# bramtoula/multi_robot_SLAM_separators

Measured on AMD Instinct MI355X. Metric: candidate keyframe-pair verifications/sec (NetVLAD NN + ORB match + RANSAC) @1/2/4/8 GPU, higher is better.
Workload: dtype u8+f16+f32+f64

## Files before the change

multi_robot_slam_separators_amd/csrc/k_ransac.hip:

```cpp
#include "sf_device_math.hpp"
#include "sf_internal.hpp"
#include "k_ba.hip"

namespace {

struct RansacLds {
  float4* src;
  float4* dst;
  float* d2;
  uint8_t* mask_a;
  uint8_t* mask_b;
  double* red;
  unsigned long long* sums;
  int* misc;
  float* hyp;
  int* hyp_cnt;
  float* best;
  float* bc;
  uint32_t* cidx;
};

__device__ __forceinline__ RansacLds ransac_carve(unsigned char* p, int kcap) {
  RansacLds L;
  L.src = (float4*)p; p += (size_t)kcap * 16;
  L.dst = (float4*)p; p += (size_t)kcap * 16;
  L.red = (double*)p; p += 64 * 8;
  L.sums = (unsigned long long*)p; p += 4 * 8;
  L.d2 = (float*)p; p += (size_t)kcap * 4;
  L.misc = (int*)p; p += 16 * 4;
  L.mask_a = p; p += kcap;
  L.mask_b = p; p += kcap;
  L.hyp = (float*)p; p += 12 * 64 * 4;
  L.hyp_cnt = (int*)p; p += 5 * 64 * 4;
  L.best = (float*)p; p += 16 * 4;
  L.bc = (float*)p; p += 16 * 4;
  L.cidx = (uint32_t*)p;
  return L;
}

__device__ __forceinline__ bool draw_sample(const RansacLds& L, uint64_t seed, uint32_t it, int max_checks,
                                            uint32_t m, double sdt, uint32_t& s0, uint32_t& s1, uint32_t& s2) {
  for (int a = 0; a < max_checks; ++a) {
    sfd::sample_triplet(seed, it, (uint32_t)a, m, s0, s1, s2);
    float4 p0 = L.src[s0], p1 = L.src[s1], p2 = L.src[s2];
    float ax = p1.x - p0.x, ay = p1.y - p0.y, az = p1.z - p0.z;
    float bx = p2.x - p0.x, by = p2.y - p0.y, bz = p2.z - p0.z;
    float cx = p2.x - p1.x, cy = p2.y - p1.y, cz = p2.z - p1.z;
    float da = (ax * ax + ay * ay) + az * az;
    float db = (bx * bx + by * by) + bz * bz;
    float dc = (cx * cx + cy * cy) + cz * cz;
    if ((double)da > sdt && (double)db > sdt && (double)dc > sdt) return true;
  }
  return false;
}

__device__ inline void fit3(const RansacLds& L, uint32_t s0, uint32_t s1, uint32_t s2, float (&coef)[12]) {
  const float4 p[3] = {L.src[s0], L.src[s1], L.src[s2]};
  const float4 q[3] = {L.dst[s0], L.dst[s1], L.dst[s2]};
  const double inv_n = 1.0 / 3.0;
  double mp[3] = {0.0, 0.0, 0.0}, mq[3] = {0.0, 0.0, 0.0};
#pragma unroll
  for (int i = 0; i < 3; ++i) {
    mp[0] += (double)p[i].x; mp[1] += (double)p[i].y; mp[2] += (double)p[i].z;
    mq[0] += (double)q[i].x; mq[1] += (double)q[i].y; mq[2] += (double)q[i].z;
  }
#pragma unroll
  for (int j = 0; j < 3; ++j) { mp[j] *= inv_n; mq[j] *= inv_n; }
  double S[3][3] = {{0.0, 0.0, 0.0}, {0.0, 0.0, 0.0}, {0.0, 0.0, 0.0}};
  double ga = 0.0, gb = 0.0;
#pragma unroll
  for (int i = 0; i < 3; ++i) {
    const double a[3] = {(double)p[i].x - mp[0], (double)p[i].y - mp[1], (double)p[i].z - mp[2]};
    const double b[3] = {(double)q[i].x - mq[0], (double)q[i].y - mq[1], (double)q[i].z - mq[2]};
#pragma unroll
    for (int j = 0; j < 3; ++j)
#pragma unroll
      for (int k = 0; k < 3; ++k) S[j][k] += a[j] * b[k];
    ga += (a[0] * a[0] + a[1] * a[1]) + a[2] * a[2];
    gb += (b[0] * b[0] + b[1] * b[1]) + b[2] * b[2];
  }
  sfd::rigid_from_moments(S, mp, mq, ga, gb, coef);
}

template <int NW>
__device__ inline void fit_masked(const RansacLds& L, int m, const uint8_t* mask, int n_in, int tid) {
  const double inv_n = 1.0 / (double)n_in;
  double s6[6];
  sfd::canon_reduce<6, 16, NW>(m, tid, L.red, s6, [&](int i, double (&a)[6]) {
    if (mask[i]) {
      float4 p = L.src[i], q = L.dst[i];
      a[0] += (double)p.x; a[1] += (double)p.y; a[2] += (double)p.z;
      a[3] += (double)q.x; a[4] += (double)q.y; a[5] += (double)q.z;
    }
  });
  double mp[3] = {s6[0] * inv_n, s6[1] * inv_n, s6[2] * inv_n};
  double mq[3] = {s6[3] * inv_n, s6[4] * inv_n, s6[5] * inv_n};
  double s9[11];
  sfd::canon_reduce<11, 16, NW>(m, tid, L.red, s9, [&](int i, double (&acc)[11]) {
    if (mask[i]) {
      float4 p = L.src[i], q = L.dst[i];
      const double a[3] = {(double)p.x - mp[0], (double)p.y - mp[1], (double)p.z - mp[2]};
      const double b[3] = {(double)q.x - mq[0], (double)q.y - mq[1], (double)q.z - mq[2]};
#pragma unroll
      for (int j = 0; j < 3; ++j)
#pragma unroll
        for (int k = 0; k < 3; ++k) acc[3 * j + k] += a[j] * b[k];
      acc[9] += (a[0] * a[0] + a[1] * a[1]) + a[2] * a[2];
      acc[10] += (b[0] * b[0] + b[1] * b[1]) + b[2] * b[2];
    }
  });
  if (tid < 64) {
    double S[3][3];
#pragma unroll
    for (int j = 0; j < 3; ++j)
#pragma unroll
      for (int k = 0; k < 3; ++k) S[j][k] = s9[3 * j + k];
    float coef[12];
    sfd::rigid_from_moments(S, mp, mq, s9[9], s9[10], coef);
    if (tid < 12) {
      float v = coef[0];
#pragma unroll
      for (int k = 1; k < 12; ++k) v = (tid == k) ? coef[k] : v;
      L.bc[tid] = v;
    }
  }
}

struct SelCounts { int n, low, diff; };

template <int NW>
__device__ inline SelCounts select_within(const RansacLds& L, int m, const float* cf, double thr2, uint8_t* mask,
                                          const uint8_t* prev, double sigma, double thr, int tid) {
  float coef[12];
#pragma unroll
  for (int k = 0; k < 12; ++k) coef[k] = cf[k];
  unsigned long long acc = 0;
  const int m4 = (m + 3) & ~3;
  for (int i = tid; i < m4; i += 64 * NW) {
    float r2 = __int_as_float(0x7F800000);
    if (i < m) {
      float4 p = L.src[i], q = L.dst[i];
      const float v = sfd::residual2(coef, p.x, p.y, p.z, q.x, q.y, q.z);
      const bool in = (double)v < thr2;
      r2 = in ? v : r2;
      const bool was = prev ? prev[i] != 0 : false;
      mask[i] = in ? 1 : 0;
      const bool low = in && !(thr < sigma * sqrt(2.1981 * (double)v));
      acc += (in ? 1ull : 0ull) + (low ? (1ull << 13) : 0ull) + ((was != in) ? (1ull << 26) : 0ull);
    }
    L.d2[i] = r2;
  }
  const int lane = tid & 63, wave = tid >> 6;
#pragma unroll
  for (int off = 32; off >= 1; off >>= 1) acc += __shfl_xor(acc, off);
  __syncthreads();
  if (lane == 0) L.sums[wave] = acc;
  __syncthreads();
  unsigned long long t = L.sums[0];
#pragma unroll
  for (int w = 1; w < NW; ++w) t += L.sums[w];
  SelCounts c;
  c.n = (int)(t & 0x1FFFull);
  c.low = (int)((t >> 13) & 0x1FFFull);
  c.diff = (int)((t >> 26) & 0x1FFFull);
  return c;
}

typedef __attribute__((address_space(3))) const float* lds_cfloat_p;
typedef __attribute__((address_space(3))) unsigned* lds_uint_p;
typedef __attribute__((address_space(3))) int* lds_int_p;
template <int NT>
__device__ __attribute__((noinline)) float radix_select_rank(lds_cfloat_p d2, lds_uint_p hist, lds_int_p misc, int m4,
                                                             int rank, int tid) {
  const int lane = tid & 63, wave = tid >> 6;
  for (int b = tid; b < 4 * 256; b += NT) hist[b] = 0u;
  __syncthreads();
  unsigned prefix = 0u;
#pragma unroll 1
  for (int p = 0; p < 4; ++p) {
    const int shift = 24 - 8 * p;
    for (int i = tid; i < m4; i += NT) {
      const unsigned bits = __float_as_uint(d2[i]);
      if (p == 0 || (bits >> (shift + 8)) == prefix)
        __hip_atomic_fetch_add(&hist[p * 256 + ((bits >> shift) & 255u)], 1u, __ATOMIC_RELAXED, __HIP_MEMORY_SCOPE_WORKGROUP);
    }
    __syncthreads();
    if (wave == 0) {
      const unsigned h0 = hist[p * 256 + 4 * lane], h1 = hist[p * 256 + 4 * lane + 1], h2 = hist[p * 256 + 4 * lane + 2],
                     h3 = hist[p * 256 + 4 * lane + 3];
      const unsigned s = (h0 + h1) + (h2 + h3);
      unsigned incl = s;
#pragma unroll
      for (int off = 1; off < 64; off <<= 1) {
        const unsigned y = __shfl_up(incl, off);
        if (lane >= off) incl += y;
      }
      const unsigned excl = incl - s;
      if (excl <= (unsigned)rank && (unsigned)rank < incl) {
        unsigned r = (unsigned)rank - excl;
        int b = 0;
        if (r >= h0) { r -= h0; b = 1; if (r >= h1) { r -= h1; b = 2; if (r >= h2) { r -= h2; b = 3; } } }
        misc[2] = (int)((prefix << 8) | (unsigned)(4 * lane + b));
        misc[3] = (int)r;
      }
    }
    __syncthreads();
    prefix = (unsigned)misc[2];
    rank = misc[3];
  }
  return __uint_as_float(prefix);
}

template <int NW>
__device__ __forceinline__ double variance_of(const RansacLds& L, int m, int n, int tid) {
  const float medv = radix_select_rank<64 * NW>((lds_cfloat_p)L.d2, (lds_uint_p) reinterpret_cast<unsigned*>(L.hyp),
                                       (lds_int_p)L.misc, (m + 3) & ~3, n >> 1, tid);
  return 2.1981 * (double)medv;
}

template <int R>
__device__ __forceinline__ int count_round(const RansacLds& L, const int* hv, int i0, int i1, int lane, float thr2f) {
  constexpr int G = 64 / R;
  const int h = lane & (R - 1), g = lane / R;
  int cnt = 0;
  if (hv[h]) {
    float coef[12];
#pragma unroll
    for (int k = 0; k < 12; ++k) coef[k] = L.hyp[k * 64 + h];
    int i = i0 + g;
#pragma unroll 1
    for (; i + 3 * G < i1; i += 4 * G) {
      float4 p[4], q[4];
#pragma unroll
      for (int u = 0; u < 4; ++u) { p[u] = L.src[i + u * G]; q[u] = L.dst[i + u * G]; }
#pragma unroll
      for (int u = 0; u < 4; ++u) {
        const float r2 = sfd::residual2(coef, p[u].x, p[u].y, p[u].z, q[u].x, q[u].y, q[u].z);
        cnt += (r2 <= thr2f) ? 1 : 0;
      }
    }
#pragma unroll 1
    for (; i < i1; i += G) {
      const float4 p = L.src[i], q = L.dst[i];
      const float r2 = sfd::residual2(coef, p.x, p.y, p.z, q.x, q.y, q.z);
      cnt += (r2 <= thr2f) ? 1 : 0;
    }
  }
  return cnt;
}

__device__ __forceinline__ int count_own(const RansacLds& L, const float (&coef)[12], int m, float thr2f) {
  int cnt = 0;
  int i = 0;
#pragma unroll 1
  for (; i + 1 < m; i += 2) {
    const float4 p0 = L.src[i], q0 = L.dst[i], p1 = L.src[i + 1], q1 = L.dst[i + 1];
    const float r0 = sfd::residual2(coef, p0.x, p0.y, p0.z, q0.x, q0.y, q0.z);
    const float r1 = sfd::residual2(coef, p1.x, p1.y, p1.z, q1.x, q1.y, q1.z);
    cnt += ((r0 <= thr2f) ? 1 : 0) + ((r1 <= thr2f) ? 1 : 0);
  }
  if (i < m) {
    const float4 p = L.src[i], q = L.dst[i];
    const float r2 = sfd::residual2(coef, p.x, p.y, p.z, q.x, q.y, q.z);
    cnt += (r2 <= thr2f) ? 1 : 0;
  }
  return cnt;
}

struct ScanState {
  int best;
  int best_it;
  int it;
  double k;
};

__device__ __forceinline__ int shfl_up_from(int v, int off, int lane) {
  const int src = lane >= off ? lane - off : lane;
  return __builtin_amdgcn_ds_bpermute(src << 2, v);
}
__device__ __forceinline__ double shfl_up_from(double v, int off, int lane) {
  const int src = lane >= off ? lane - off : lane;
  const long long b = __double_as_longlong(v);
  const int lo = __builtin_amdgcn_ds_bpermute(src << 2, (int)(b & 0xFFFFFFFFll));
  const int hi = __builtin_amdgcn_ds_bpermute(src << 2, (int)(b >> 32));
  return __longlong_as_double(((long long)hi << 32) | (unsigned)lo);
}

__device__ __forceinline__ bool replay_round(const RansacLds& L, ScanState& S, int base, int R, int lane, int c,
                                             bool present, int max_it, bool adaptive, double inv_m,
                                             double log_probability, bool park = true) {
  int x = present ? c : -1;
#pragma unroll
  for (int off = 1; off < 64; off <<= 1) {
    const int y = shfl_up_from(x, off, lane);
    if (lane >= off) x = max(x, y);
  }
  x = max(x, S.best);
  double kj = 1.0;
  if (x >= 0) {
    const double w = (double)x * inv_m;
    double pno = 1.0 - (w * w) * w;
    if (pno < 2.220446049250313e-16) pno = 2.220446049250313e-16;
    if (pno > 1.0 - 2.220446049250313e-16) pno = 1.0 - 2.220446049250313e-16;
    kj = log_probability / sfd::canon_log(pno);
  }
  double kprev = shfl_up_from(kj, 1, lane);
  if (lane == 0) kprev = S.k;
  const int it = base + lane;
  const bool top_ok = present && (!adaptive || (double)it < kprev) && c >= 0;
  const unsigned long long fail = ~__ballot(top_ok);
  const int n_proc = fail ? (__ffsll((long long)fail) - 1) : 64;
  if (n_proc > 0) {
    const int nb = __builtin_amdgcn_readlane(x, n_proc - 1);
    const long long kb = __double_as_longlong(kj);
    const double nk = __longlong_as_double(
        ((long long)__builtin_amdgcn_readlane((int)(kb >> 32), n_proc - 1) << 32) |
        (unsigned)__builtin_amdgcn_readlane((int)(kb & 0xFFFFFFFFll), n_proc - 1));
    if (nb > S.best) {
      const unsigned long long at = __ballot(present && c == nb && lane < n_proc);
      const int lb = __ffsll((long long)at) - 1;
      S.best = nb;
      S.best_it = base + lb;
      if (park && lane < 12) L.best[lane] = L.hyp[lane * 64 + lb];
    }
    S.k = nk;
  }
  S.it = base + n_proc;
  return n_proc < R || base + R > max_it;
}

__host__ __device__ inline size_t sf_ransac_lds_bytes_dev(int kcap) {
  return (size_t)kcap * 32 + 64 * 8 + 4 * 8 + (size_t)kcap * 4 + 16 * 4 + (size_t)kcap * 2 + 12 * 64 * 4 + 5 * 64 * 4 +
         16 * 4 + 16 * 4 + (size_t)kcap * 4;
}

__device__ __forceinline__ void write_null_pass(PassState& out, int matches) {
  PassState ps;
#pragma unroll
  for (int i = 0; i < 12; ++i) ps.T[i] = 0.f;
  ps.var = 1.0; ps.var_ang = 1.0;
  ps.is_null = 1;
  ps.inliers = 0;
  ps.matches = matches;
  ps.pad = 0;
  out = ps;
}

template <int DIR = 0, int NW = 4>
__device__ __forceinline__ void ransac_body(const StoreView& st, int pair, int sF, int sT, const uint32_t* cl, int n_corr,
                                            PassState& out, const DeviceParams& P, unsigned char* lds,
                                            int trace_base = 2, uint8_t* mask_out = nullptr) {
  constexpr int NT = 64 * NW;
  const int tid = (int)threadIdx.x;
  const int lane = tid & 63, wave = tid >> 6;
  const int kcap = st.kcap;
  const RansacLds L = ransac_carve(lds, kcap);

  const float* xF = st.xyz + (size_t)sF * kcap * 3;
  const float* xT = st.xyz + (size_t)sT * kcap * 3;
  if (tid < 16) L.misc[tid] = 0;
  __syncthreads();
  int m = 0;
  for (int base = 0; base < n_corr; base += NT) {
    const int i = base + tid;
    bool ok = false;
    float ax = 0, ay = 0, az = 0, bx = 0, by = 0, bz = 0;
    if (i < n_corr) {
      const uint32_t c = cl[i];
      const float* a = DIR ? xT + 3 * (c >> 16) : xF + 3 * (c & 0xFFFFu);
      const float* b = DIR ? xF + 3 * (c & 0xFFFFu) : xT + 3 * (c >> 16);
      ax = a[0]; ay = a[1]; az = a[2];
      bx = b[0]; by = b[1]; bz = b[2];
      ok = sfd::finite3(ax, ay, az) && sfd::finite3(bx, by, bz) && (ax != 0.f || ay != 0.f || az != 0.f) &&
           (bx != 0.f || by != 0.f || bz != 0.f);
    }
    const unsigned long long bal = __ballot(ok);
    const int before = __popcll(bal & ((1ull << lane) - 1ull));
    if (lane == 0) L.misc[4 + wave] = __popcll(bal);
    __syncthreads();
    int woff = 0, total = 0;
#pragma unroll
    for (int w = 0; w < NW; ++w) {
      int c = L.misc[4 + w];
      if (w < wave) woff += c;
      total += c;
    }
    if (ok) {
      L.src[m + woff + before] = make_float4(ax, ay, az, 0.f);
      L.dst[m + woff + before] = make_float4(bx, by, bz, 0.f);
      L.cidx[m + woff + before] = cl[i];
    }
    m += total;
    __syncthreads();
  }

  SF_TRACE_MARK(P, pair, trace_base + 0);
  if (m < P.min_inliers || m < 3) {
    if (tid == 0) write_null_pass(out, m);
    return;
  }

  const int fit_wave = pair & (NW - 1);

  const double inv_m = 1.0 / (double)m;
  if (tid == 0) reinterpret_cast<double*>(L.sums)[2] = inv_m;
  double sdt = 0.0;
  {
    double mean[3];
    double s3[3];
    sfd::canon_reduce<3, 16, NW>(m, tid, L.red, s3, [&](int i, double (&a)[3]) {
      float4 p = L.src[i];
      a[0] += (double)p.x; a[1] += (double)p.y; a[2] += (double)p.z;
    });
    mean[0] = s3[0] * inv_m; mean[1] = s3[1] * inv_m; mean[2] = s3[2] * inv_m;
    double c6[6];
    sfd::canon_reduce<6, 16, NW>(m, tid, L.red, c6, [&](int i, double (&a)[6]) {
      float4 p = L.src[i];
      const double a0 = (double)p.x - mean[0], a1 = (double)p.y - mean[1], a2 = (double)p.z - mean[2];
      a[0] += a0 * a0; a[1] += a0 * a1; a[2] += a0 * a2;
      a[3] += a1 * a1; a[4] += a1 * a2; a[5] += a2 * a2;
    });
    if (wave == fit_wave) {
      double ev[3];
      sfd::sym3_eigenvalues(c6[0] * inv_m, c6[1] * inv_m, c6[2] * inv_m, c6[3] * inv_m, c6[4] * inv_m, c6[5] * inv_m, ev);
      sdt = ((sqrt(ev[0]) + sqrt(ev[1])) + sqrt(ev[2])) / 3.0;
      sdt = sdt * sdt;
      if (lane == 0) {
        double* st = reinterpret_cast<double*>(L.sums);
        st[0] = sdt;
        st[1] = 1.0;
        L.misc[12] = -1;
        L.misc[13] = -1;
        L.misc[14] = 0;
      }
    }
  }

  if (P.dbg_stop == 1) { if (tid == 0) write_null_pass(out, m); return; }
  SF_TRACE_MARK(P, pair, trace_base + 1);

  const int max_it = P.iterations;
  int* hv = L.hyp_cnt + 4 * 64;
  {
    constexpr int R = 16;
    const int base = 0;
    int lane_r = lane, wave_r = wave;
    asm volatile("" : "+v"(lane_r), "+v"(wave_r));
    const int it = base + lane_r;
    if (wave_r == fit_wave) {
      int valid = 0;
      if (lane_r < R && it <= max_it) {
        uint32_t s0, s1, s2;
        if (draw_sample(L, P.seed, (uint32_t)it, P.max_sample_checks, (uint32_t)m, reinterpret_cast<const double*>(L.sums)[0],
                        s0, s1, s2)) {
          float coef[12];
          fit3(L, s0, s1, s2, coef);
          int lane_s = lane;
          asm volatile("" : "+v"(lane_s));
#pragma unroll
          for (int k = 0; k < 12; ++k) L.hyp[k * 64 + lane_s] = coef[k];
          valid = 1;
        }
      }
      int lane_s = lane;
      asm volatile("" : "+v"(lane_s));
      hv[lane_s] = valid;
    }
    __syncthreads();
    SF_TRACE_MARK(P, pair, trace_base == 2 ? 18 : 21);
    {
      int lane_c = lane, wave_c = wave;
      asm volatile("" : "+v"(lane_c), "+v"(wave_c));
      const double thr2 = P.inlier_thr * P.inlier_thr;
      float thr2f = (float)thr2;
      if ((double)thr2f >= thr2) thr2f = __uint_as_float(__float_as_uint(thr2f) - 1u);
      const int slice = (m + NW - 1) / NW;
      const int i0 = min(m, wave_c * slice), i1 = min(m, i0 + slice);
      L.hyp_cnt[wave_c * 64 + lane_c] = count_round<16>(L, hv, i0, i1, lane_c, thr2f);
    }
    __syncthreads();
    SF_TRACE_MARK(P, pair, trace_base == 2 ? 19 : 22);
    if (wave_r == fit_wave) {
      asm volatile("" : "+v"(lane_r));
      int tot = 0;
      const int h = lane_r & 15;
#pragma unroll
      for (int w = 0; w < NW; ++w)
#pragma unroll
        for (int g = 0; g < 4; ++g) tot += L.hyp_cnt[w * 64 + g * 16 + h];
      const bool present = lane_r < R && it <= max_it;
      const int c = (present && hv[lane_r]) ? tot : -1;
      ScanState S;
      S.best = L.misc[12]; S.best_it = L.misc[13]; S.it = L.misc[14];
      S.k = reinterpret_cast<const double*>(L.sums)[1];
      const bool stop = replay_round(L, S, base, R, lane_r, c, present, max_it, P.adaptive_stop != 0,
                                     reinterpret_cast<const double*>(L.sums)[2],
                                     sfd::canon_log(1.0 - 0.99));
      if (lane_r == 0) {
        L.misc[12] = S.best; L.misc[13] = S.best_it; L.misc[14] = S.it;
        reinterpret_cast<double*>(L.sums)[1] = S.k;
        L.misc[0] = S.best_it;
        L.misc[1] = stop ? 1 : 0;
      }
    }
    __syncthreads();
    SF_TRACE_MARK(P, pair, trace_base == 2 ? 20 : 23);
  }
  if (!L.misc[1]) {
    for (int base = 16; base <= max_it; base += 64 * NW) {
      int lane_r = lane, wave_r = wave;
      asm volatile("" : "+v"(lane_r), "+v"(wave_r));
      const int it = base + 64 * wave_r + lane_r;
      float coef[12];
#pragma unroll
      for (int k = 0; k < 12; ++k) coef[k] = 0.f;
      int cnt = -1;
      if (it <= max_it) {
        uint32_t s0, s1, s2;
        if (draw_sample(L, P.seed, (uint32_t)it, P.max_sample_checks, (uint32_t)m, reinterpret_cast<const double*>(L.sums)[0],
                        s0, s1, s2)) {
          fit3(L, s0, s1, s2, coef);
          const double thr2 = P.inlier_thr * P.inlier_thr;
          float thr2f = (float)thr2;
          if ((double)thr2f >= thr2) thr2f = __uint_as_float(__float_as_uint(thr2f) - 1u);
          cnt = count_own(L, coef, m, thr2f);
        }
      }
      {
        int lane_s = lane, wave_s = wave;
        asm volatile("" : "+v"(lane_s), "+v"(wave_s));
        L.hyp_cnt[wave_s * 64 + lane_s] = cnt;
      }
      __syncthreads();
      if (wave_r == fit_wave) {
        asm volatile("" : "+v"(lane_r));
        ScanState S;
        S.best = L.misc[12]; S.best_it = L.misc[13]; S.it = L.misc[14];
        S.k = reinterpret_cast<const double*>(L.sums)[1];
        bool stop = false;
#pragma unroll 1
        for (int sub = 0; sub < NW && !stop; ++sub) {
          const int b = base + 64 * sub;
          if (b > max_it) break;
          const bool present = b + lane_r <= max_it;
          const int c = present ? L.hyp_cnt[sub * 64 + lane_r] : -1;
          stop = replay_round(L, S, b, 64, lane_r, c, present, max_it, P.adaptive_stop != 0,
                              reinterpret_cast<const double*>(L.sums)[2], sfd::canon_log(1.0 - 0.99), false);
        }
        if (lane_r == 0) {
          L.misc[12] = S.best; L.misc[13] = S.best_it; L.misc[14] = S.it;
          reinterpret_cast<double*>(L.sums)[1] = S.k;
          L.misc[0] = S.best_it;
          L.misc[1] = stop ? 1 : 0;
        }
      }
      __syncthreads();
      if (cnt >= 0 && L.misc[0] == it) {
#pragma unroll
        for (int k = 0; k < 12; ++k) L.best[k] = coef[k];
      }
      __syncthreads();
      if (L.misc[1]) break;
    }
  }
  int tid_b = tid;
  asm volatile("" : "+v"(tid_b));
  if (P.dbg_stop == 2 || P.dbg_stop == 3) { if (tid_b == 0) write_null_pass(out, m); return; }
  SF_TRACE_MARK(P, pair, trace_base + 2);
  const int best_it = L.misc[0];
  if (best_it < 0) {
    if (tid_b == 0) write_null_pass(out, m);
    return;
  }

  const double thr = P.inlier_thr;
  const double thr2 = thr * thr;
  const double sigma = P.refine_sigma;
  SelCounts sc = select_within<NW>(L, m, L.best, thr2, L.mask_a, nullptr, sigma, thr, tid_b);
  int n_inl = sc.n;
  const uint8_t* inl = L.mask_a;
  int n_last = n_inl;
  const float* model = L.best;

  if (P.dbg_stop == 4) { if (tid_b == 0) write_null_pass(out, m); return; }
  SF_TRACE_MARK(P, pair, trace_base + 3);

  if (P.refine_iterations > 0) {
    double error_threshold = thr;
    int refine_iterations = 0;
    bool inlier_changed = false;
    uint8_t* prev = L.mask_a;
    uint8_t* neu = L.mask_b;
    int n_prev = n_inl, n_new = 0;
    for (int i = tid_b; i < m; i += NT) neu[i] = 0;
    if (tid_b < 12) L.bc[tid_b] = L.best[tid_b];
    int n_sizes = 0, z1 = 0, z2 = 0, z3 = 0, z4 = 0;
    do {
      if (n_prev >= 3) fit_masked<NW>(L, m, prev, n_prev, tid_b);
      z4 = z3; z3 = z2; z2 = z1; z1 = n_prev;
      ++n_sizes;
      __syncthreads();
      sc = select_within<NW>(L, m, L.bc, error_threshold * error_threshold, neu, prev, sigma, thr, tid_b);
      n_new = sc.n;
      n_last = n_new;
      if (n_new == 0) {
        ++refine_iterations;
        if (refine_iterations >= P.refine_iterations) break;
        continue;
      }
      if ((n_new >> 1) < sc.low) {
        const double variance = variance_of<NW>(L, m, n_new, tid_b);
        const double sthr = sigma * sqrt(variance);
        error_threshold = thr < sthr ? thr : sthr;
      } else {
        error_threshold = thr;
      }
      inlier_changed = false;
      { uint8_t* t = prev; prev = neu; neu = t; int tn = n_prev; n_prev = n_new; n_new = tn; }
      if (n_new != n_prev) {
        if (n_sizes >= 4 && z1 == z3 && z2 == z4) break;
        inlier_changed = true;
        continue;
      }
      inlier_changed = sc.diff != 0;
    } while (inlier_changed && ++refine_iterations < P.refine_iterations);
    inl = neu;
    n_inl = n_new;
    model = L.bc;
  }

  if (P.dbg_stop == 5) { if (tid_b == 0) write_null_pass(out, m); return; }
  SF_TRACE_MARK(P, pair, trace_base + 4);
  if (n_inl >= 3) {
    if (mask_out)
      for (int i = tid; i < m; i += NT)
        if (inl[i]) mask_out[L.cidx[i] & 0xFFFFu] = 1;
    const double variance = variance_of<NW>(L, m, n_last, tid_b);
    if (tid_b == 0) {
      PassState ps;
#pragma unroll
      for (int i = 0; i < 12; ++i) ps.T[i] = 0.f;
      ps.is_null = 1;
      ps.matches = m;
      ps.pad = 0;
      ps.var = variance;
      ps.var_ang = variance;
      ps.inliers = n_inl;
      if (n_inl >= P.min_inliers) {
        double R9[9], t[3];
#pragma unroll
        for (int i = 0; i < 3; ++i) {
#pragma unroll
          for (int j = 0; j < 3; ++j) R9[3 * i + j] = (double)model[4 * i + j];
          t[i] = (double)model[4 * i + 3];
        }
        bool allz = true;
#pragma unroll
        for (int i = 0; i < 3; ++i) {
#pragma unroll
          for (int j = 0; j < 3; ++j) ps.T[4 * i + j] = (float)R9[3 * j + i];
          ps.T[4 * i + 3] = (float)(-((R9[i] * t[0] + R9[3 + i] * t[1]) + R9[6 + i] * t[2]));
        }
#pragma unroll
        for (int i = 0; i < 12; ++i) allz = allz && (ps.T[i] == 0.f);
        ps.is_null = allz ? 1 : 0;
        if (P.force_3dof && !allz) sfd::to3dof_canon(ps.T);
      }
      out = ps;
    }
  } else if (tid_b == 0) {
    write_null_pass(out, m);
  }
  SF_TRACE_MARK(P, pair, trace_base + 5);
}

__device__ inline void pass_to3dof(PassState& ps, int times) {
  if (ps.is_null) return;
  for (int t = 0; t < times; ++t) sfd::to3dof_canon(ps.T);
}

template <int DIR>
__global__ void __launch_bounds__(SF_BLOCK, 4)
k_ransac(StoreView st, const int32_t* __restrict__ pair_from, const int32_t* __restrict__ pair_to,
         const int32_t* __restrict__ list, const int32_t* __restrict__ counter,
         const uint32_t* __restrict__ corr, const CorrHeader* __restrict__ hdr,
         PassState* __restrict__ pass, uint8_t* __restrict__ mask, int extra_3dof, DeviceParams P) {
  if ((int)blockIdx.x >= *counter) return;
  extern __shared__ __attribute__((aligned(16))) unsigned char smem_raw[];
  const int pair = list[blockIdx.x];
  ransac_body<DIR>(st, pair, pair_from[pair], pair_to[pair], corr + (size_t)pair * st.kcap, hdr[pair].n_corr,
                       pass[pair], P, smem_raw, 2, mask ? mask + (size_t)pair * st.kcap : nullptr);
  if (extra_3dof && threadIdx.x == 0) pass_to3dof(pass[pair], extra_3dof);
}

__global__ void __launch_bounds__(64)
k_merge_directions(const int32_t* __restrict__ list, const int32_t* __restrict__ counter, PassState* __restrict__ fwd,
                   const PassState* __restrict__ back, const uint8_t* __restrict__ mask_f,
                   const uint8_t* __restrict__ mask_b, int kcap, int extra_3dof) {
  if ((int)blockIdx.x >= *counter) return;
  const int pair = list[blockIdx.x], lane = threadIdx.x;
  int uni = 0;
  for (int i = lane; i < kcap; i += 64) uni += (mask_f[(size_t)pair * kcap + i] | mask_b[(size_t)pair * kcap + i]) ? 1 : 0;
#pragma unroll
  for (int off = 32; off >= 1; off >>= 1) uni += __shfl_xor(uni, off);
  if (lane != 0) return;
  PassState a = fwd[pair];
  const PassState b = back[pair];
  a.inliers = uni;
  a.matches = a.matches > b.matches ? a.matches : b.matches;
  if (!b.is_null) {
    float inv[12];
    sfd::rigid_inverse_canon(b.T, inv);
    if (a.is_null) {
#pragma unroll
      for (int i = 0; i < 12; ++i) a.T[i] = inv[i];
      a.is_null = 0;
      a.var = b.var;
      a.var_ang = b.var_ang;
    } else {
      float mid[12];
      sfd::interpolate_half_canon(a.T, inv, mid);
#pragma unroll
      for (int i = 0; i < 12; ++i) a.T[i] = mid[i];
      a.var = (a.var + b.var) / 2.0;
      a.var_ang = (a.var_ang + b.var_ang) / 2.0;
    }
  }
  pass_to3dof(a, extra_3dof);
  fwd[pair] = a;
}

}

size_t sf_ransac_lds_bytes(int kcap, int iterations) {
  (void)iterations;
  return sf_ransac_lds_bytes_dev(kcap);
}

int sf_launch_ransac(sf_context* c, StoreView st, const int32_t* d_from, const int32_t* d_to, int n, int pass) {
  if (n <= 0) return SF_OK;
  const bool ba = c->dparams.bundle_adjustment != 0;
  const size_t lds = (sf_ransac_lds_bytes(st.kcap, c->dparams.iterations) + 15) & ~(size_t)15;
  if (lds > 160 * 1024) return sf_fail(c, SF_ERANGE, "RANSAC workgroup needs %zu B of LDS (> 160 KiB)", lds);
  const bool bidir = c->dparams.bidirectional != 0;
  bool& attr = c->ransac_attr_set;
  if (!attr) {
    SF_HIP(c, hipFuncSetAttribute((const void*)k_ransac<0>, hipFuncAttributeMaxDynamicSharedMemorySize, 160 * 1024));
    SF_HIP(c, hipFuncSetAttribute((const void*)k_ransac<1>, hipFuncAttributeMaxDynamicSharedMemorySize, 160 * 1024));
    attr = true;
  }
  int32_t* counters = (int32_t*)c->w->counters.p;
  const int32_t* list = (const int32_t*)(pass == 1 ? c->w->list1.p : c->w->list3.p);
  const int32_t* counter = counters + (pass == 1 ? 0 : 2);
  PassState* ps = (PassState*)(pass == 1 ? c->w->pass1.p : c->w->pass2.p);
  const int end_3dof = c->dparams.force_3dof ? (pass == 1 ? 2 : 1) : 0;
  uint8_t *mask_f = nullptr, *mask_b = nullptr;
  if (bidir) {
    int rc;
    const size_t mb = (size_t)n * st.kcap;
    if ((rc = sf_buf_reserve(c, c->w->dir_mask, 2 * mb)) != SF_OK) return rc;
    if ((rc = sf_buf_reserve(c, c->w->pass_back, (size_t)n * sizeof(PassState))) != SF_OK) return rc;
    mask_f = (uint8_t*)c->w->dir_mask.p;
    mask_b = mask_f + mb;
    SF_HIP(c, hipMemsetAsync(mask_f, 0, 2 * mb, c->stream));
  } else if (ba) {
    int rc;
    const size_t mb = (size_t)n * st.kcap;
    if ((rc = sf_buf_reserve(c, c->w->dir_mask, mb)) != SF_OK) return rc;
    mask_f = (uint8_t*)c->w->dir_mask.p;
    SF_HIP(c, hipMemsetAsync(mask_f, 0, mb, c->stream));
  }
  const int kid = pass == 1 ? SF_K_RANSAC1 : SF_K_RANSAC2;
  sf_prof_begin(c, kid);
  auto launch = [&](auto kern, PassState* out, uint8_t* mask, int extra) {
    hipLaunchKernelGGL(kern, dim3(n), dim3(SF_BLOCK), lds, c->stream, st, d_from, d_to, list, counter,
                       (const uint32_t*)(pass == 1 ? c->w->corr1.p : c->w->corr2.p),
                       (const CorrHeader*)(pass == 1 ? c->w->hdr1.p : c->w->hdr2.p), out, mask, extra, c->dparams);
  };
  if (ba && !bidir) launch(k_ransac<0>, ps, mask_f, 0);
  else if (!bidir) launch(k_ransac<0>, ps, nullptr, end_3dof);
  else {
    launch(k_ransac<0>, ps, mask_f, 0);
    launch(k_ransac<1>, (PassState*)c->w->pass_back.p, mask_b, 0);
    if (ba) {
      const int rc = sf_launch_merge_directions_ba(c, st, d_from, d_to, n, pass, false, mask_f, mask_b);
      if (rc != SF_OK) return rc;
    } else
    hipLaunchKernelGGL(k_merge_directions, dim3(n), dim3(64), 0, c->stream, list, counter, ps,
                       (const PassState*)c->w->pass_back.p, (const uint8_t*)mask_f, (const uint8_t*)mask_b, st.kcap, end_3dof);
  }
  sf_prof_end(c, kid);
  SF_HIP(c, hipGetLastError());
  if (ba && !bidir) return sf_launch_ba_pass(c, st, d_from, d_to, n, pass, pass == 1 ? 1 : 3, mask_f, nullptr, false, nullptr);
  return SF_OK;
}
```

multi_robot_slam_separators_amd/csrc/sf_device_math.hpp:

```cpp
#pragma once
#include <hip/hip_runtime.h>
#include <stdint.h>

namespace sfd {

__device__ __forceinline__ uint64_t mix64(uint64_t z) {
  z += 0x9E3779B97F4A7C15ULL;
  z = (z ^ (z >> 30)) * 0xBF58476D1CE4E5B9ULL;
  z = (z ^ (z >> 27)) * 0x94D049BB133111EBULL;
  return z ^ (z >> 31);
}

__device__ __forceinline__ void sample_triplet(uint64_t seed, uint32_t it, uint32_t attempt, uint32_t m,
                                               uint32_t& i0, uint32_t& i1, uint32_t& i2) {
  uint64_t ha = mix64(seed ^ mix64(((uint64_t)it << 32) | (uint64_t)attempt));
  uint64_t hb = mix64(ha);
  uint32_t r0 = (uint32_t)(ha >> 32), r1 = (uint32_t)ha, r2 = (uint32_t)(hb >> 32);
  i0 = __umulhi(r0, m);
  i1 = __umulhi(r1, m - 1);
  if (i1 >= i0) ++i1;
  i2 = __umulhi(r2, m - 2);
  uint32_t lo = i0 < i1 ? i0 : i1, hi = i0 < i1 ? i1 : i0;
  if (i2 >= lo) ++i2;
  if (i2 >= hi) ++i2;
}

__device__ inline double canon_log(double x) {
  int e;
  double m = frexp(x, &e);
  if (m < 0.70710678118654752440) { m = m * 2.0; e -= 1; }
  double z = (m - 1.0) / (m + 1.0);
  double z2 = z * z;
  double s = 1.0 / 27.0;
#pragma unroll
  for (int k = 12; k >= 0; --k) s = s * z2 + 1.0 / (double)(2 * k + 1);
  return 2.0 * z * s + (double)e * 0.69314718055994530942;
}

template <int N>
__device__ inline void jacobi(double (&a)[N][N], double (&v)[N][N]) {
#pragma unroll
  for (int i = 0; i < N; ++i)
#pragma unroll
    for (int j = 0; j < N; ++j) v[i][j] = (i == j) ? 1.0 : 0.0;
  for (int sweep = 0; sweep < 50; ++sweep) {
    double sm = 0.0;
#pragma unroll
    for (int p = 0; p < N - 1; ++p)
#pragma unroll
      for (int q = p + 1; q < N; ++q) sm += fabs(a[p][q]);
    if (sm == 0.0) break;
#pragma unroll
    for (int p = 0; p < N - 1; ++p) {
#pragma unroll
      for (int q = p + 1; q < N; ++q) {
        double apq = a[p][q];
        double g = 100.0 * fabs(apq);
        double app = fabs(a[p][p]), aqq = fabs(a[q][q]);
        if (sweep > 3 && app + g == app && aqq + g == aqq) {
          a[p][q] = 0.0;
          a[q][p] = 0.0;
        } else if (apq != 0.0) {
          double h = a[q][q] - a[p][p];
          double t;
          if (fabs(h) + g == fabs(h)) {
            t = apq / h;
          } else {
            double theta = 0.5 * h / apq;
            t = 1.0 / (fabs(theta) + sqrt(1.0 + theta * theta));
            if (theta < 0.0) t = -t;
          }
          double c = 1.0 / sqrt(1.0 + t * t);
          double s = t * c;
#pragma unroll
          for (int k = 0; k < N; ++k) {
            double akp = a[k][p], akq = a[k][q];
            a[k][p] = c * akp - s * akq;
            a[k][q] = s * akp + c * akq;
          }
#pragma unroll
          for (int k = 0; k < N; ++k) {
            double apk = a[p][k], aqk = a[q][k];
            a[p][k] = c * apk - s * aqk;
            a[q][k] = s * apk + c * aqk;
          }
          a[p][q] = 0.0;
          a[q][p] = 0.0;
#pragma unroll
          for (int k = 0; k < N; ++k) {
            double vkp = v[k][p], vkq = v[k][q];
            v[k][p] = c * vkp - s * vkq;
            v[k][q] = s * vkp + c * vkq;
          }
        }
      }
    }
  }
}

__device__ __forceinline__ double det3(double a, double b, double c, double d, double e, double f, double g,
                                       double h, double i) {
  return (a * (e * i - f * h) - b * (d * i - f * g)) + c * (d * h - e * g);
}

__device__ inline void sym3_eigenvalues(double c00, double c01, double c02, double c11, double c12, double c22,
                                        double (&ev)[3]) {
  const double c2 = (c00 + c11) + c22;
  const double c1 = ((c00 * c11 - c01 * c01) + (c00 * c22 - c02 * c02)) + (c11 * c22 - c12 * c12);
  const double c0 = det3(c00, c01, c02, c01, c11, c12, c02, c12, c22);
  double x = c2;
  for (int it = 0; it < 50; ++it) {
    const double pv = ((x - c2) * x + c1) * x - c0;
    const double dp = (3.0 * x - 2.0 * c2) * x + c1;
    if (dp == 0.0) break;
    const double xn = x - pv / dp;
    if (!(xn < x)) break;
    const double step = x - xn;
    x = xn;
    if (step <= 1e-14 * fabs(xn)) break;
  }
  const double l1 = x > 0.0 ? x : 0.0;
  const double s = c2 - l1;
  const double q = c1 - l1 * s;
  double disc = s * s - 4.0 * q;
  if (!(disc > 0.0)) disc = 0.0;
  const double r = sqrt(disc);
  double l2 = 0.5 * (s + r), l3 = 0.5 * (s - r);
  if (!(l2 > 0.0)) l2 = 0.0;
  if (!(l3 > 0.0)) l3 = 0.0;
  ev[0] = l1; ev[1] = l2; ev[2] = l3;
}

__device__ inline void rigid_from_moments(const double (&S)[3][3], const double (&mp)[3],
                                          const double (&mq)[3], double ga, double gb, float (&coef)[12]) {
  double Nm[4][4];
  Nm[0][0] = (S[0][0] + S[1][1]) + S[2][2];
  Nm[1][1] = (S[0][0] - S[1][1]) - S[2][2];
  Nm[2][2] = (S[1][1] - S[0][0]) - S[2][2];
  Nm[3][3] = (S[2][2] - S[0][0]) - S[1][1];
  Nm[0][1] = Nm[1][0] = S[1][2] - S[2][1];
  Nm[0][2] = Nm[2][0] = S[2][0] - S[0][2];
  Nm[0][3] = Nm[3][0] = S[0][1] - S[1][0];
  Nm[1][2] = Nm[2][1] = S[0][1] + S[1][0];
  Nm[1][3] = Nm[3][1] = S[2][0] + S[0][2];
  Nm[2][3] = Nm[3][2] = S[1][2] + S[2][1];

  double ss = 0.0;
#pragma unroll
  for (int j = 0; j < 3; ++j)
#pragma unroll
    for (int k = 0; k < 3; ++k) ss += S[j][k] * S[j][k];
  const double c2 = -2.0 * ss;
  const double c1 = -8.0 * det3(S[0][0], S[0][1], S[0][2], S[1][0], S[1][1], S[1][2], S[2][0], S[2][1], S[2][2]);
  const double m0 = det3(Nm[1][1], Nm[1][2], Nm[1][3], Nm[2][1], Nm[2][2], Nm[2][3], Nm[3][1], Nm[3][2], Nm[3][3]);
  const double m1 = det3(Nm[1][0], Nm[1][2], Nm[1][3], Nm[2][0], Nm[2][2], Nm[2][3], Nm[3][0], Nm[3][2], Nm[3][3]);
  const double m2 = det3(Nm[1][0], Nm[1][1], Nm[1][3], Nm[2][0], Nm[2][1], Nm[2][3], Nm[3][0], Nm[3][1], Nm[3][3]);
  const double m3 = det3(Nm[1][0], Nm[1][1], Nm[1][2], Nm[2][0], Nm[2][1], Nm[2][2], Nm[3][0], Nm[3][1], Nm[3][2]);
  const double c0 = ((Nm[0][0] * m0 - Nm[0][1] * m1) + Nm[0][2] * m2) - Nm[0][3] * m3;

  double x = 0.5 * (ga + gb);
  for (int it = 0; it < 50; ++it) {
    const double x2 = x * x;
    const double b = (x2 + c2) * x;
    const double a = b + c1;
    const double pv = a * x + c0;
    const double dp = (2.0 * x2 * x + b) + a;
    if (dp == 0.0) break;
    const double xn = x - pv / dp;
    if (!(xn < x)) break;
    const double step = x - xn;
    x = xn;
    if (step <= 1e-14 * fabs(xn)) break;
  }

  const double b00 = Nm[0][0] - x, b11 = Nm[1][1] - x, b22 = Nm[2][2] - x, b33 = Nm[3][3] - x;
  const double b01 = Nm[0][1], b02 = Nm[0][2], b03 = Nm[0][3], b12 = Nm[1][2], b13 = Nm[1][3], b23 = Nm[2][3];
  const double a00 = det3(b11, b12, b13, b12, b22, b23, b13, b23, b33);
  const double a11 = det3(b00, b02, b03, b02, b22, b23, b03, b23, b33);
  const double a22 = det3(b00, b01, b03, b01, b11, b13, b03, b13, b33);
  const double a33 = det3(b00, b01, b02, b01, b11, b12, b02, b12, b22);
  const double a01 = -det3(b01, b12, b13, b02, b22, b23, b03, b23, b33);
  const double a02 = det3(b01, b11, b13, b02, b12, b23, b03, b13, b33);
  const double a03 = -det3(b01, b11, b12, b02, b12, b22, b03, b13, b23);
  const double a12 = -det3(b00, b01, b03, b02, b12, b23, b03, b13, b33);
  const double a13 = det3(b00, b01, b02, b02, b12, b22, b03, b13, b23);
  const double a23 = -det3(b00, b01, b02, b01, b11, b12, b03, b13, b23);
  double best = fabs(a00);
  double w = a00, qx = a01, qy = a02, qz = a03;
  if (fabs(a11) > best) { best = fabs(a11); w = a01; qx = a11; qy = a12; qz = a13; }
  if (fabs(a22) > best) { best = fabs(a22); w = a02; qx = a12; qy = a22; qz = a23; }
  if (fabs(a33) > best) { best = fabs(a33); w = a03; qx = a13; qy = a23; qz = a33; }
  double nrm2 = ((w * w + qx * qx) + qy * qy) + qz * qz;
  if (!(best > 0.0) || !(nrm2 > 0.0) || !isfinite(nrm2)) {
    const double shift = 0.5 * (ga + gb);
    double v0 = 1.0, v1 = 0.5, v2 = 0.25, v3 = 0.125;
    for (int it = 0; it < 64; ++it) {
      const double u0 = (((Nm[0][0] + shift) * v0 + Nm[0][1] * v1) + Nm[0][2] * v2) + Nm[0][3] * v3;
      const double u1 = ((Nm[0][1] * v0 + (Nm[1][1] + shift) * v1) + Nm[1][2] * v2) + Nm[1][3] * v3;
      const double u2 = ((Nm[0][2] * v0 + Nm[1][2] * v1) + (Nm[2][2] + shift) * v2) + Nm[2][3] * v3;
      const double u3 = ((Nm[0][3] * v0 + Nm[1][3] * v1) + Nm[2][3] * v2) + (Nm[3][3] + shift) * v3;
      const double n2 = ((u0 * u0 + u1 * u1) + u2 * u2) + u3 * u3;
      if (!(n2 > 0.0) || !isfinite(n2)) break;
      const double in = 1.0 / sqrt(n2);
      v0 = u0 * in; v1 = u1 * in; v2 = u2 * in; v3 = u3 * in;
    }
    w = v0; qx = v1; qy = v2; qz = v3;
    nrm2 = ((w * w + qx * qx) + qy * qy) + qz * qz;
  }
  const double inv = 1.0 / sqrt(nrm2);
  w = w * inv;
  const double x_ = qx * inv, y = qy * inv, z = qz * inv;
  const double xx = x_ * x_, yy = y * y, zz = z * z, xy = x_ * y, xz = x_ * z, yz = y * z;
  const double wx = w * x_, wy = w * y, wz = w * z;
  double R[9];
  R[0] = 1.0 - 2.0 * (yy + zz); R[1] = 2.0 * (xy - wz);       R[2] = 2.0 * (xz + wy);
  R[3] = 2.0 * (xy + wz);       R[4] = 1.0 - 2.0 * (xx + zz); R[5] = 2.0 * (yz - wx);
  R[6] = 2.0 * (xz - wy);       R[7] = 2.0 * (yz + wx);       R[8] = 1.0 - 2.0 * (xx + yy);
#pragma unroll
  for (int j = 0; j < 3; ++j) {
    double t = mq[j] - ((R[3 * j] * mp[0] + R[3 * j + 1] * mp[1]) + R[3 * j + 2] * mp[2]);
    coef[4 * j + 0] = (float)R[3 * j + 0];
    coef[4 * j + 1] = (float)R[3 * j + 1];
    coef[4 * j + 2] = (float)R[3 * j + 2];
    coef[4 * j + 3] = (float)t;
  }
}

__device__ __forceinline__ float residual2(const float (&c)[12], float px, float py, float pz,
                                           float qx, float qy, float qz) {
  float tx = __fmaf_rn(c[2], pz, __fmaf_rn(c[1], py, __fmaf_rn(c[0], px, c[3])));
  float ty = __fmaf_rn(c[6], pz, __fmaf_rn(c[5], py, __fmaf_rn(c[4], px, c[7])));
  float tz = __fmaf_rn(c[10], pz, __fmaf_rn(c[9], py, __fmaf_rn(c[8], px, c[11])));
  float dx = tx - qx, dy = ty - qy, dz = tz - qz;
  return __fmaf_rn(dz, dz, __fmaf_rn(dy, dy, dx * dx));
}


template <int C>
__device__ __forceinline__ void sum_stage(double (&w)[32], int& idx, int lane, int off) {
  if constexpr (C > 1) {
    const bool up = (lane & off) != 0;
#pragma unroll
    for (int k = 0; k < C / 2; ++k) {
      const double send = up ? w[k] : w[k + C / 2];
      const double keep = up ? w[k + C / 2] : w[k];
      w[k] = keep + __shfl_xor(send, off);
    }
    idx += up ? C / 2 : 0;
  } else {
    w[0] = w[0] + __shfl_xor(w[0], off);
  }
}

template <int N, int STRIDE>
__device__ __forceinline__ void block_sum_canon(double (&v)[N], double* red, int tid) {
  static_assert(N >= 1 && N <= 32 && STRIDE >= N, "at most 32 values");
  constexpr int P = N <= 1 ? 1 : N <= 2 ? 2 : N <= 4 ? 4 : N <= 8 ? 8 : N <= 16 ? 16 : 32;
  static_assert(STRIDE >= P, "scratch rows must hold the padded count");
  const int lane = tid & 63, wave = tid >> 6;
  double w[32];
#pragma unroll
  for (int k = 0; k < 32; ++k) w[k] = k < N ? v[k] : 0.0;
  int idx = 0;
  sum_stage<P>(w, idx, lane, 32);
  sum_stage<(P / 2 > 1 ? P / 2 : 1)>(w, idx, lane, 16);
  sum_stage<(P / 4 > 1 ? P / 4 : 1)>(w, idx, lane, 8);
  sum_stage<(P / 8 > 1 ? P / 8 : 1)>(w, idx, lane, 4);
  sum_stage<(P / 16 > 1 ? P / 16 : 1)>(w, idx, lane, 2);
  sum_stage<(P / 32 > 1 ? P / 32 : 1)>(w, idx, lane, 1);
  __syncthreads();
  red[wave * STRIDE + idx] = w[0];
  __syncthreads();
#pragma unroll
  for (int k = 0; k < N; ++k) v[k] = ((red[k] + red[STRIDE + k]) + red[2 * STRIDE + k]) + red[3 * STRIDE + k];
}

template <int N, int STRIDE, int NW, class F>
__device__ __forceinline__ void canon_reduce(int m, int tid, double* red, double (&out)[N], F acc) {
  if constexpr (NW == 4) {
#pragma unroll
    for (int k = 0; k < N; ++k) out[k] = 0.0;
    for (int i = tid; i < m; i += 256) acc(i, out);
    block_sum_canon<N, STRIDE>(out, red, tid);
  } else {
    static_assert(NW == 1 || NW == 2, "one, two or four wavefronts");
    constexpr int P = N <= 1 ? 1 : N <= 2 ? 2 : N <= 4 ? 4 : N <= 8 ? 8 : N <= 16 ? 16 : 32;
    static_assert(STRIDE >= P, "scratch rows must hold the padded count");
    const int lane = tid & 63, wave = tid >> 6;
    __syncthreads();
#pragma unroll 1
    for (int j = 0; j < 4 / NW; ++j) {
      const int vw = wave * (4 / NW) + j;
      if (64 * vw >= m) {
        if (lane < P) red[vw * STRIDE + lane] = 0.0;
        continue;
      }
      double w[32];
#pragma unroll
      for (int k = 0; k < 32; ++k) w[k] = 0.0;
      {
        double v[N];
#pragma unroll
        for (int k = 0; k < N; ++k) v[k] = 0.0;
        for (int i = lane + 64 * vw; i < m; i += 256) acc(i, v);
#pragma unroll
        for (int k = 0; k < N; ++k) w[k] = v[k];
      }
      int idx = 0;
      sum_stage<P>(w, idx, lane, 32);
      sum_stage<(P / 2 > 1 ? P / 2 : 1)>(w, idx, lane, 16);
      sum_stage<(P / 4 > 1 ? P / 4 : 1)>(w, idx, lane, 8);
      sum_stage<(P / 8 > 1 ? P / 8 : 1)>(w, idx, lane, 4);
      sum_stage<(P / 16 > 1 ? P / 16 : 1)>(w, idx, lane, 2);
      sum_stage<(P / 32 > 1 ? P / 32 : 1)>(w, idx, lane, 1);
      red[vw * STRIDE + idx] = w[0];
    }
    __syncthreads();
#pragma unroll
    for (int k = 0; k < N; ++k) out[k] = ((red[k] + red[STRIDE + k]) + red[2 * STRIDE + k]) + red[3 * STRIDE + k];
  }
}

template <int N, int STRIDE>
__device__ __forceinline__ void block_sum_canon_to_lds(const double (&v)[N], double* red, double* out, int tid) {
  static_assert(N >= 1 && N <= 32 && STRIDE >= N, "at most 32 values");
  constexpr int P = N <= 1 ? 1 : N <= 2 ? 2 : N <= 4 ? 4 : N <= 8 ? 8 : N <= 16 ? 16 : 32;
  static_assert(STRIDE >= P, "scratch rows must hold the padded count");
  const int lane = tid & 63, wave = tid >> 6;
  double w[32];
#pragma unroll
  for (int k = 0; k < 32; ++k) w[k] = k < N ? v[k] : 0.0;
  int idx = 0;
  sum_stage<P>(w, idx, lane, 32);
  sum_stage<(P / 2 > 1 ? P / 2 : 1)>(w, idx, lane, 16);
  sum_stage<(P / 4 > 1 ? P / 4 : 1)>(w, idx, lane, 8);
  sum_stage<(P / 8 > 1 ? P / 8 : 1)>(w, idx, lane, 4);
  sum_stage<(P / 16 > 1 ? P / 16 : 1)>(w, idx, lane, 2);
  sum_stage<(P / 32 > 1 ? P / 32 : 1)>(w, idx, lane, 1);
  __syncthreads();
  red[wave * STRIDE + idx] = w[0];
  __syncthreads();
  if (tid < N) out[tid] = ((red[tid] + red[STRIDE + tid]) + red[2 * STRIDE + tid]) + red[3 * STRIDE + tid];
  __syncthreads();
}

template <int N, int STRIDE, int NW, bool ONCE = false, class F>
__device__ __forceinline__ void canon_reduce_to_lds(int m, int tid, double* red, double* out, F acc) {
  if constexpr (NW == 4) {
    double v[N];
#pragma unroll
    for (int k = 0; k < N; ++k) v[k] = 0.0;
    if constexpr (ONCE) { if (tid < m) acc(tid, v); }
    else { for (int i = tid; i < m; i += 256) acc(i, v); }
    block_sum_canon_to_lds<N, STRIDE>(v, red, out, tid);
  } else {
    static_assert(NW == 1 || NW == 2, "one, two or four wavefronts");
    constexpr int P = N <= 1 ? 1 : N <= 2 ? 2 : N <= 4 ? 4 : N <= 8 ? 8 : N <= 16 ? 16 : 32;
    static_assert(STRIDE >= P, "scratch rows must hold the padded count");
    const int lane = tid & 63, wave = tid >> 6;
    __syncthreads();
#pragma unroll 1
    for (int j = 0; j < 4 / NW; ++j) {
      const int vw = wave * (4 / NW) + j;
      if (64 * vw >= m) {
        if (lane < P) red[vw * STRIDE + lane] = 0.0;
        continue;
      }
      double w[32];
#pragma unroll
      for (int k = 0; k < 32; ++k) w[k] = 0.0;
      {
        double v[N];
#pragma unroll
        for (int k = 0; k < N; ++k) v[k] = 0.0;
        if constexpr (ONCE) { if (lane + 64 * vw < m) acc(lane + 64 * vw, v); }
        else { for (int i = lane + 64 * vw; i < m; i += 256) acc(i, v); }
#pragma unroll
        for (int k = 0; k < N; ++k) w[k] = v[k];
      }
      int idx = 0;
      sum_stage<P>(w, idx, lane, 32);
      sum_stage<(P / 2 > 1 ? P / 2 : 1)>(w, idx, lane, 16);
      sum_stage<(P / 4 > 1 ? P / 4 : 1)>(w, idx, lane, 8);
      sum_stage<(P / 8 > 1 ? P / 8 : 1)>(w, idx, lane, 4);
      sum_stage<(P / 16 > 1 ? P / 16 : 1)>(w, idx, lane, 2);
      sum_stage<(P / 32 > 1 ? P / 32 : 1)>(w, idx, lane, 1);
      red[vw * STRIDE + idx] = w[0];
    }
    __syncthreads();
    if (tid < N) out[tid] = ((red[tid] + red[STRIDE + tid]) + red[2 * STRIDE + tid]) + red[3 * STRIDE + tid];
    __syncthreads();
  }
}

__device__ __forceinline__ bool finite3(float x, float y, float z) {
  return isfinite(x) && isfinite(y) && isfinite(z);
}

__device__ inline void to3dof_canon(float* T) {
  const double r11 = (double)T[0], r21 = (double)T[4];
  const double h = sqrt(r11 * r11 + r21 * r21);
  float c = 1.0f, s = 0.0f;
  if (h > 0.0) { c = (float)(r11 / h); s = (float)(r21 / h); }
  const float x = T[3], y = T[7];
  T[0] = c; T[1] = -s; T[2] = 0.0f; T[3] = x;
  T[4] = s; T[5] = c; T[6] = 0.0f; T[7] = y;
  T[8] = 0.0f; T[9] = 0.0f; T[10] = 1.0f; T[11] = 0.0f;
}

__device__ inline void quat_from_rot_canon(const float* T, double (&q)[4]) {
  double m[3][3];
#pragma unroll
  for (int i = 0; i < 3; ++i)
#pragma unroll
    for (int j = 0; j < 3; ++j) m[i][j] = (double)T[4 * i + j];
  const double tr = (m[0][0] + m[1][1]) + m[2][2];
  if (tr > 0.0) {
    double t = sqrt(tr + 1.0);
    q[3] = 0.5 * t; t = 0.5 / t;
    q[0] = (m[2][1] - m[1][2]) * t; q[1] = (m[0][2] - m[2][0]) * t; q[2] = (m[1][0] - m[0][1]) * t;
  } else {
    int i = 0;
    if (m[1][1] > m[0][0]) i = 1;
    if (m[2][2] > m[i][i]) i = 2;
    const int j = (i + 1) % 3, k = (j + 1) % 3;
    double t = sqrt(((m[i][i] - m[j][j]) - m[k][k]) + 1.0);
    double qv[3];
    qv[i] = 0.5 * t; t = 0.5 / t;
    q[3] = (m[k][j] - m[j][k]) * t;
    qv[j] = (m[j][i] + m[i][j]) * t;
    qv[k] = (m[k][i] + m[i][k]) * t;
    q[0] = qv[0]; q[1] = qv[1]; q[2] = qv[2];
  }
}

__device__ inline void rigid_inverse_canon(const float* T, float* out) {
  double R[9], t[3];
#pragma unroll
  for (int i = 0; i < 3; ++i) {
#pragma unroll
    for (int j = 0; j < 3; ++j) R[3 * i + j] = (double)T[4 * i + j];
    t[i] = (double)T[4 * i + 3];
  }
#pragma unroll
  for (int i = 0; i < 3; ++i) {
#pragma unroll
    for (int j = 0; j < 3; ++j) out[4 * i + j] = (float)R[3 * j + i];
    out[4 * i + 3] = (float)(-((R[i] * t[0] + R[3 + i] * t[1]) + R[6 + i] * t[2]));
  }
}

__device__ inline void interpolate_half_canon(const float* A, const float* B, float* out) {
  double qa[4], qb[4], q[4];
  quat_from_rot_canon(A, qa);
  quat_from_rot_canon(B, qb);
  const double d = ((qa[0] * qb[0] + qa[1] * qb[1]) + qa[2] * qb[2]) + qa[3] * qb[3];
#pragma unroll
  for (int i = 0; i < 4; ++i) q[i] = d < 0.0 ? qa[i] - qb[i] : qa[i] + qb[i];
  const double n = sqrt(((q[0] * q[0] + q[1] * q[1]) + q[2] * q[2]) + q[3] * q[3]);
  const double x = q[0] / n, y = q[1] / n, z = q[2] / n, w = q[3] / n;
  const double tx = 2.0 * x, ty = 2.0 * y, tz = 2.0 * z;
  const double twx = tx * w, twy = ty * w, twz = tz * w, txx = tx * x, txy = ty * x, txz = tz * x, tyy = ty * y,
               tyz = tz * y, tzz = tz * z;
  out[0] = (float)(1.0 - (tyy + tzz)); out[1] = (float)(txy - twz);         out[2] = (float)(txz + twy);
  out[4] = (float)(txy + twz);         out[5] = (float)(1.0 - (txx + tzz)); out[6] = (float)(tyz - twx);
  out[8] = (float)(txz - twy);         out[9] = (float)(tyz + twx);         out[10] = (float)(1.0 - (txx + tyy));
#pragma unroll
  for (int i = 0; i < 3; ++i) out[4 * i + 3] = A[4 * i + 3] + 0.5f * (B[4 * i + 3] - A[4 * i + 3]);
}

}
```

Measured before the change: 24.98 million.

## Add wave-ballot radix select, precomputed low-residual boundary, and skip idle reduction work

For small correspondence sets (at most 256), the rank selection now runs a single-wave bitwise ballot search instead of the 4-pass LDS histogram radix select. The per-point sqrt-based 'low residual' test is replaced by a float threshold precomputed once per pair, which falls back to the exact rule when the boundary cannot be confirmed. Block reductions skip the shuffle tree for wavefronts with no elements, and only the consuming waves fold the final sums. This trims per-iteration ALU and LDS-atomic work, at the cost of extra code paths and a more fragile equivalence argument.

```diff
diff --git a/multi_robot_slam_separators_amd/csrc/k_ransac.hip b/multi_robot_slam_separators_amd/csrc/k_ransac.hip
--- a/multi_robot_slam_separators_amd/csrc/k_ransac.hip
+++ b/multi_robot_slam_separators_amd/csrc/k_ransac.hip
@@ -108,7 +108,7 @@
       acc[9] += (a[0] * a[0] + a[1] * a[1]) + a[2] * a[2];
       acc[10] += (b[0] * b[0] + b[1] * b[1]) + b[2] * b[2];
     }
-  });
+  }, tid < 64);
   if (tid < 64) {
     double S[3][3];
 #pragma unroll
@@ -128,6 +128,23 @@
 
 struct SelCounts { int n, low, diff; };
 
+__device__ __forceinline__ bool low_rule(float v, double thr, double sigma) {
+  return !(thr < sigma * sqrt(2.1981 * (double)v));
+}
+__device__ inline void low_boundary(const RansacLds& L, double thr, double sigma, int lane) {
+  const double q = thr / sigma;
+  const float c = (float)((q * q) / 2.1981);
+  const unsigned cb = __float_as_uint(c);
+  bool have = c > 0.f && cb >= 32u && cb + 31u < 0x7F800000u;
+  const float cand = __uint_as_float(have ? cb - 32u + (unsigned)lane : 0u);
+  const unsigned long long ok = __ballot(low_rule(cand, thr, sigma));
+  have = have && ok != 0ull && ok != ~0ull && (ok & (ok + 1ull)) == 0ull;
+  if (lane == 0) {
+    L.misc[8] = have ? (int)(cb - 32u + (unsigned)__popcll(ok) - 1u) : 0;
+    L.misc[9] = have ? 1 : 0;
+  }
+}
+
 template <int NW>
 __device__ inline SelCounts select_within(const RansacLds& L, int m, const float* cf, double thr2, uint8_t* mask,
                                           const uint8_t* prev, double sigma, double thr, int tid) {
@@ -136,6 +153,8 @@
   for (int k = 0; k < 12; ++k) coef[k] = cf[k];
   unsigned long long acc = 0;
   const int m4 = (m + 3) & ~3;
+  const bool have_low = L.misc[9] != 0;
+  const float v_low = __int_as_float(L.misc[8]);
   for (int i = tid; i < m4; i += 64 * NW) {
     float r2 = __int_as_float(0x7F800000);
     if (i < m) {
@@ -145,7 +164,7 @@
       r2 = in ? v : r2;
       const bool was = prev ? prev[i] != 0 : false;
       mask[i] = in ? 1 : 0;
-      const bool low = in && !(thr < sigma * sqrt(2.1981 * (double)v));
+      const bool low = in && (have_low ? v <= v_low : low_rule(v, thr, sigma));
       acc += (in ? 1ull : 0ull) + (low ? (1ull << 13) : 0ull) + ((was != in) ? (1ull << 26) : 0ull);
     }
     L.d2[i] = r2;
@@ -169,10 +188,34 @@
 typedef __attribute__((address_space(3))) const float* lds_cfloat_p;
 typedef __attribute__((address_space(3))) unsigned* lds_uint_p;
 typedef __attribute__((address_space(3))) int* lds_int_p;
+typedef float lds_float4_v __attribute__((ext_vector_type(4)));
 template <int NT>
 __device__ __attribute__((noinline)) float radix_select_rank(lds_cfloat_p d2, lds_uint_p hist, lds_int_p misc, int m4,
                                                              int rank, int tid) {
   const int lane = tid & 63, wave = tid >> 6;
+  m4 = __builtin_amdgcn_readfirstlane(m4);
+  rank = __builtin_amdgcn_readfirstlane(rank);
+  if (m4 <= 256) {
+    __syncthreads();
+    if (wave == 0) {
+      uint4 e = make_uint4(0x7F800000u, 0x7F800000u, 0x7F800000u, 0x7F800000u);
+      if (4 * lane < m4) {
+        const lds_float4_v f = *reinterpret_cast<__attribute__((address_space(3))) const lds_float4_v*>(d2 + 4 * lane);
+        e = make_uint4(__float_as_uint(f.x), __float_as_uint(f.y), __float_as_uint(f.z), __float_as_uint(f.w));
+      }
+      unsigned prefix = 0u;
+#pragma unroll
+      for (int bit = 31; bit >= 0; --bit) {
+        const unsigned t = prefix | (1u << bit);
+        const int below = (__popcll(__ballot(e.x < t)) + __popcll(__ballot(e.y < t))) +
+                          (__popcll(__ballot(e.z < t)) + __popcll(__ballot(e.w < t)));
+        prefix = below <= rank ? t : prefix;
+      }
+      if (lane == 0) misc[2] = (int)prefix;
+    }
+    __syncthreads();
+    return __uint_as_float((unsigned)misc[2]);
+  }
   for (int b = tid; b < 4 * 256; b += NT) hist[b] = 0u;
   __syncthreads();
   unsigned prefix = 0u;
@@ -419,7 +462,7 @@
       const double a0 = (double)p.x - mean[0], a1 = (double)p.y - mean[1], a2 = (double)p.z - mean[2];
       a[0] += a0 * a0; a[1] += a0 * a1; a[2] += a0 * a2;
       a[3] += a1 * a1; a[4] += a1 * a2; a[5] += a2 * a2;
-    });
+    }, wave == fit_wave);
     if (wave == fit_wave) {
       double ev[3];
       sfd::sym3_eigenvalues(c6[0] * inv_m, c6[1] * inv_m, c6[2] * inv_m, c6[3] * inv_m, c6[4] * inv_m, c6[5] * inv_m, ev);
@@ -433,6 +476,7 @@
         L.misc[13] = -1;
         L.misc[14] = 0;
       }
+      low_boundary(L, P.inlier_thr, P.refine_sigma, lane);
     }
   }
 
diff --git a/multi_robot_slam_separators_amd/csrc/sf_device_math.hpp b/multi_robot_slam_separators_amd/csrc/sf_device_math.hpp
--- a/multi_robot_slam_separators_amd/csrc/sf_device_math.hpp
+++ b/multi_robot_slam_separators_amd/csrc/sf_device_math.hpp
@@ -253,35 +253,43 @@
 }
 
 template <int N, int STRIDE>
-__device__ __forceinline__ void block_sum_canon(double (&v)[N], double* red, int tid) {
+__device__ __forceinline__ void block_sum_canon(double (&v)[N], double* red, int tid, bool empty = false,
+                                                bool fold = true) {
   static_assert(N >= 1 && N <= 32 && STRIDE >= N, "at most 32 values");
   constexpr int P = N <= 1 ? 1 : N <= 2 ? 2 : N <= 4 ? 4 : N <= 8 ? 8 : N <= 16 ? 16 : 32;
   static_assert(STRIDE >= P, "scratch rows must hold the padded count");
   const int lane = tid & 63, wave = tid >> 6;
-  double w[32];
-#pragma unroll
-  for (int k = 0; k < 32; ++k) w[k] = k < N ? v[k] : 0.0;
-  int idx = 0;
-  sum_stage<P>(w, idx, lane, 32);
-  sum_stage<(P / 2 > 1 ? P / 2 : 1)>(w, idx, lane, 16);
-  sum_stage<(P / 4 > 1 ? P / 4 : 1)>(w, idx, lane, 8);
-  sum_stage<(P / 8 > 1 ? P / 8 : 1)>(w, idx, lane, 4);
-  sum_stage<(P / 16 > 1 ? P / 16 : 1)>(w, idx, lane, 2);
-  sum_stage<(P / 32 > 1 ? P / 32 : 1)>(w, idx, lane, 1);
+  double w0 = 0.0;
+  int idx = lane & (P - 1);
+  if (!empty) {
+    double w[32];
+#pragma unroll
+    for (int k = 0; k < 32; ++k) w[k] = k < N ? v[k] : 0.0;
+    idx = 0;
+    sum_stage<P>(w, idx, lane, 32);
+    sum_stage<(P / 2 > 1 ? P / 2 : 1)>(w, idx, lane, 16);
+    sum_stage<(P / 4 > 1 ? P / 4 : 1)>(w, idx, lane, 8);
+    sum_stage<(P / 8 > 1 ? P / 8 : 1)>(w, idx, lane, 4);
+    sum_stage<(P / 16 > 1 ? P / 16 : 1)>(w, idx, lane, 2);
+    sum_stage<(P / 32 > 1 ? P / 32 : 1)>(w, idx, lane, 1);
+    w0 = w[0];
+  }
   __syncthreads();
-  red[wave * STRIDE + idx] = w[0];
+  red[wave * STRIDE + idx] = w0;
   __syncthreads();
-#pragma unroll
-  for (int k = 0; k < N; ++k) v[k] = ((red[k] + red[STRIDE + k]) + red[2 * STRIDE + k]) + red[3 * STRIDE + k];
+  if (fold) {
+#pragma unroll
+    for (int k = 0; k < N; ++k) v[k] = ((red[k] + red[STRIDE + k]) + red[2 * STRIDE + k]) + red[3 * STRIDE + k];
+  }
 }
 
 template <int N, int STRIDE, int NW, class F>
-__device__ __forceinline__ void canon_reduce(int m, int tid, double* red, double (&out)[N], F acc) {
+__device__ __forceinline__ void canon_reduce(int m, int tid, double* red, double (&out)[N], F acc, bool fold = true) {
   if constexpr (NW == 4) {
 #pragma unroll
     for (int k = 0; k < N; ++k) out[k] = 0.0;
     for (int i = tid; i < m; i += 256) acc(i, out);
-    block_sum_canon<N, STRIDE>(out, red, tid);
+    block_sum_canon<N, STRIDE>(out, red, tid, 64 * __builtin_amdgcn_readfirstlane(tid >> 6) >= m, fold);
   } else {
     static_assert(NW == 1 || NW == 2, "one, two or four wavefronts");
     constexpr int P = N <= 1 ? 1 : N <= 2 ? 2 : N <= 4 ? 4 : N <= 8 ? 8 : N <= 16 ? 16 : 32;
@@ -316,8 +324,13 @@
       red[vw * STRIDE + idx] = w[0];
     }
     __syncthreads();
-#pragma unroll
-    for (int k = 0; k < N; ++k) out[k] = ((red[k] + red[STRIDE + k]) + red[2 * STRIDE + k]) + red[3 * STRIDE + k];
+    if (fold) {
+#pragma unroll
+      for (int k = 0; k < N; ++k) out[k] = ((red[k] + red[STRIDE + k]) + red[2 * STRIDE + k]) + red[3 * STRIDE + k];
+    } else {
+#pragma unroll
+      for (int k = 0; k < N; ++k) out[k] = 0.0;
+    }
   }
 }
 
```

Result: no change. 25.09 million, median of 6 (+0.4%).
